# YessionCC/AR-NeRF

Measured on AMD Instinct MI355X. Metric: training rays/sec + test PSNR, Lego 8192-ray batch, 1/2/4/8 MI355X, higher is better.
Workload: dtype fp16 field (MLP forward, backward and weight gradients on fp16 MFMA operands, fp32 accumulate) / fp32 march, composite, Adam; 1 GPU; lego-shaped training step: 8192 rays/rank, scale 0.5, 1 x 128^3 grid, L=16 F=2 T=2^19 hash, 64-wide MLPs, raw loss, Adam lr 1e-2; batch_rays_per_gpu=8192, global_batch_rays=8192, pretrain_steps=2000, graphs=True, chunk_first=64, row_forward=1, march_fork=r1, parallelism=dp1, hash_backward=hybrid, bin_level_lo=8, bin_merge_hi=11, steps_per_graph_replay=2, erode=False

## Files before the change

ar-nerf_amd/csrc/hashbin.hip:

```cpp
#pragma clang fp contract(off)

#include "common.h"
#include "grid.h"

namespace ngp {

constexpr int BSHIFT = 13, BENT = 1 << BSHIFT;
constexpr int NBL = (1 << 19) / BENT;
constexpr int ACC_T = BENT / 8;
constexpr int NSLOT = L * NBL;
constexpr int MAXB = 2048;
constexpr int TILE = 256;
constexpr int RPT = TILE * 4 / 256;
constexpr uint32_t CH = 32768;
constexpr uint32_t IB_CAP = 8192;
constexpr uint32_t F_C0 = 1u << 28;
constexpr uint32_t F_SINGLE = 1u << 29;

struct BinArgs {
    int lo;
    uint32_t merge;
    uint32_t bbase[L + 1];
    int64_t tiles_cap;
};

struct BinWs {
    uint32_t* fb;
    uint32_t* tot;
    uint32_t* rstart;
    uint32_t* items;
    uint32_t* ib;
    uint32_t* ofs;
    uint4* rec;
};

static size_t align256(size_t x) { return (x + 255) & ~(size_t)255; }

static size_t bin_ws_bytes(int64_t tiles, BinWs* w, void* base) {
    const size_t o_fb = 0, o_tot = align256((MAXB + 1) * 4), o_rs = o_tot + align256(MAXB * 4),
                 o_it = o_rs + align256((MAXB + 1) * 4), o_ib = o_it + align256((MAXB + 1) * 4),
                 o_ofs = o_ib + align256(IB_CAP * 4);
    const size_t o_rec = align256(o_ofs + (size_t)tiles * NSLOT * 4);
    const size_t total = o_rec + (size_t)tiles * TILE * 4 * L * sizeof(uint4);
    if (w) {
        char* b = reinterpret_cast<char*>(base);
        w->fb = reinterpret_cast<uint32_t*>(b + o_fb);
        w->tot = reinterpret_cast<uint32_t*>(b + o_tot);
        w->rstart = reinterpret_cast<uint32_t*>(b + o_rs);
        w->items = reinterpret_cast<uint32_t*>(b + o_it);
        w->ib = reinterpret_cast<uint32_t*>(b + o_ib);
        w->ofs = reinterpret_cast<uint32_t*>(b + o_ofs);
        w->rec = reinterpret_cast<uint4*>(b + o_rec);
    }
    return total;
}

__device__ __forceinline__ void add_pair_direct(float* __restrict__ grad, uint32_t e, float w, float a0, float a1) {
    atomicAdd(grad + 2 * (size_t)e, w * a0);
    atomicAdd(grad + 2 * (size_t)e + 1, w * a1);
}

struct Rec {
    uint32_t e0, e1;
    float fx, a0, a1;
};

__device__ __forceinline__ Rec make_rec(const float in[3], float2 gd, int cy, int cz, const LevelLds& lv, int l) {
    const float sc = lv.scale[l];
    const uint32_t res = lv.res[l], size = lv.size[l];
    const bool dense = (lv.dense >> l) & 1u, pow2 = (lv.pow2 >> l) & 1u;
    float pos[3];
    uint32_t pg[3];
    level_cell(sc, in, pg, pos);
    const float wyz = (cy ? pos[1] : 1 - pos[1]) * (cz ? pos[2] : 1 - pos[2]);
    Rec r;
    r.fx = pos[0];
    r.a0 = wyz * gd.x;
    r.a1 = wyz * gd.y;
    r.e0 = corner_index(pg[0], pg[1] + cy, pg[2] + cz, res, size, dense, pow2);
    r.e1 = corner_index(pg[0] + 1, pg[1] + cy, pg[2] + cz, res, size, dense, pow2);
    return r;
}

struct RunInfo {
    bool head, longrun;
    uint64_t heads;
};
__device__ __forceinline__ RunInfo run_info(bool valid, uint32_t e0, uint32_t e1) {
    const int lane = threadIdx.x & 63;
    const uint32_t k0 = valid ? e0 : 0xffffffffu, k1 = valid ? e1 : (0xfffffff0u | (uint32_t)lane);
    const uint32_t p0 = __shfl_up(k0, 4, 64), p1 = __shfl_up(k1, 4, 64);
    RunInfo r;
    r.head = lane < 4 || !valid || p0 != k0 || p1 != k1;
    r.heads = __ballot(r.head);
    r.longrun = r.head && valid && lane + 4 < 64 && !((r.heads >> (lane + 4)) & 1ull);
    return r;
}

__device__ __forceinline__ void tile_inputs(const float* __restrict__ xyzs, const int32_t* __restrict__ sidx,
                                            const GridArgs& ga, int64_t j0, int64_t N, float in[RPT][3],
                                            bool valid[RPT]) {
    const int t = threadIdx.x;
#pragma unroll
    for (int k = 0; k < RPT; ++k) {
        const int64_t j = j0 + k * 64 + (t >> 2);
        valid[k] = j < N;
        const int64_t i = valid[k] && sidx ? (int64_t)sidx[j] : j;
        load_x01(xyzs, i, valid[k], ga, in[k]);
    }
}

__global__ void __launch_bounds__(256) hash_count_kernel(const float* __restrict__ xyzs, int64_t n,
                                                         const int64_t* __restrict__ n_dev,
                                                         const int32_t* __restrict__ sidx, GridArgs ga, BinArgs ba,
                                                         BinWs ws) {
    __shared__ LevelLds lv;
    __shared__ uint32_t cnt[NSLOT];
    NGP_PROBE_BEGIN(NGP_P_HASH_COUNT);
    load_levels(ga, lv);
    const int64_t N = ngp_capped_count(n_dev, n);
    const int64_t ntiles = min((N + TILE - 1) / TILE, ba.tiles_cap);
    const int t = threadIdx.x, yz = t & 3, cy = yz & 1, cz = yz >> 1;
    const float2 g0 = make_float2(0.f, 0.f);
    if (blockIdx.x == 0)
        for (int i = t; i <= MAXB; i += blockDim.x) ws.fb[i] = 0u;
    for (int64_t tile = blockIdx.x; tile < ntiles; tile += gridDim.x) {
        for (int i = t; i < NSLOT; i += 256) cnt[i] = 0;
        __syncthreads();
        float in[RPT][3];
        bool valid[RPT];
        tile_inputs(xyzs, sidx, ga, tile * TILE, N, in, valid);
#pragma unroll 1
        for (int l = ba.lo; l < L; ++l) {
            const bool merge = (ba.merge >> l) & 1u;
#pragma unroll
            for (int k = 0; k < RPT; ++k) {
                const Rec r = make_rec(in[k], g0, cy, cz, lv, l);
                if (merge) {
                    const RunInfo ri = run_info(valid[k], r.e0, r.e1);
                    if (!valid[k] || !ri.head) continue;
                    atomicAdd(&cnt[l * NBL + (r.e0 >> BSHIFT)], 1u);
                    if (ri.longrun) atomicAdd(&cnt[l * NBL + (r.e1 >> BSHIFT)], 1u);
                    continue;
                }
                if (!valid[k]) continue;
                atomicAdd(&cnt[l * NBL + (r.e0 >> BSHIFT)], 1u);
            }
        }
        __syncthreads();
        for (int i = t; i < NSLOT; i += 256) ws.ofs[(size_t)i * ba.tiles_cap + tile] = cnt[i];
        __syncthreads();
    }
    NGP_PROBE_END();
}

__global__ void __launch_bounds__(256) hash_scan_kernel(const int64_t* __restrict__ n_dev, int64_t n, BinArgs ba,
                                                        BinWs ws) {
    __shared__ uint32_t wsum[4];
    const int slot = blockIdx.x, l = slot / NBL, lb = slot % NBL;
    if (lb >= (int)(ba.bbase[l + 1] - ba.bbase[l])) return;
    const int64_t N = ngp_capped_count(n_dev, n);
    const int64_t ntiles = min((N + TILE - 1) / TILE, ba.tiles_cap);
    const int t = threadIdx.x, lane = t & 63, w = t >> 6;
    uint32_t carry = 0;
    for (int64_t c0 = 0; c0 < ntiles; c0 += 256) {
        const int64_t tile = c0 + t;
        uint32_t* p = ws.ofs + (size_t)slot * ba.tiles_cap + tile;
        const uint32_t v = tile < ntiles ? *p : 0u;
        uint32_t x = v;
#pragma unroll
        for (int o = 1; o < 64; o <<= 1) {
            const uint32_t y = __shfl_up(x, o, 64);
            if (lane >= o) x += y;
        }
        if (lane == 63) wsum[w] = x;
        __syncthreads();
        uint32_t before = carry;
        for (int i = 0; i < w; ++i) before += wsum[i];
        const uint32_t blk = wsum[0] + wsum[1] + wsum[2] + wsum[3];
        if (tile < ntiles) *p = before + x - v;
        carry += blk;
        __syncthreads();
    }
    if (t == 0) ws.tot[ba.bbase[l] + lb] = carry;
}

__global__ void __launch_bounds__(MAXB / 2) hash_plan_kernel(uint32_t nbt, BinWs ws) {
    __shared__ uint32_t a[MAXB / 2], c[MAXB / 2];
    NGP_PROBE_BEGIN(NGP_P_HASH_PLAN);
    const uint32_t t = threadIdx.x, b0 = 2 * t, b1 = 2 * t + 1;
    const uint32_t t0 = b0 < nbt ? ws.tot[b0] : 0u, t1 = b1 < nbt ? ws.tot[b1] : 0u;
    const uint32_t c0 = (t0 + CH - 1) / CH, c1 = (t1 + CH - 1) / CH;
    a[t] = t0 + t1;
    c[t] = c0 + c1;
    __syncthreads();
    for (uint32_t o = 1; o < MAXB / 2; o <<= 1) {
        const uint32_t va = t >= o ? a[t - o] : 0u, vc = t >= o ? c[t - o] : 0u;
        __syncthreads();
        a[t] += va;
        c[t] += vc;
        __syncthreads();
    }
    ws.rstart[b0 + 1] = a[t] - t1;
    ws.rstart[b1 + 1] = a[t];
    ws.items[b0 + 1] = c[t] - c1;
    ws.items[b1 + 1] = c[t];
    if (t == 0) { ws.rstart[0] = 0; ws.items[0] = 0; }
    for (uint32_t it = c[t] - c1 - c0; it < c[t] - c1 && it < IB_CAP; ++it) ws.ib[it] = b0;
    for (uint32_t it = c[t] - c1; it < c[t] && it < IB_CAP; ++it) ws.ib[it] = b1;
    NGP_PROBE_END();
}

template <int MODE>
__global__ void __launch_bounds__(256) hash_write_kernel(const float* __restrict__ xyzs, int64_t n,
                                                         const int64_t* __restrict__ n_dev,
                                                         const int32_t* __restrict__ sidx, GridArgs ga, BinArgs ba,
                                                         const float* __restrict__ denc, float* __restrict__ grad,
                                                         BinWs ws) {
    static_assert((MODE & 2) || NBL == 64, "MODE 0 (diagnostics) scans one wave of buckets");
    __shared__ LevelLds lv;
    __shared__ uint32_t base[NSLOT];
    __shared__ uint32_t hist2[2][NBL], loff[NBL + 1];
    __shared__ uint4 stage[TILE * 4];
    __shared__ uint8_t sbk[TILE * 4];
    uint32_t* const hall = reinterpret_cast<uint32_t*>(stage);
    static_assert(sizeof(stage) >= NSLOT * sizeof(uint32_t), "stage[] holds the per-level counters");
    NGP_PROBE_BEGIN(NGP_P_HASH_WRITE);
    load_levels(ga, lv);
    const int64_t N = ngp_capped_count(n_dev, n);
    const int64_t ntiles = (N + TILE - 1) / TILE;
    const int t = threadIdx.x, yz = t & 3, cy = yz & 1, cz = yz >> 1;
    for (int64_t tile = blockIdx.x; tile < ntiles; tile += gridDim.x) {
        const bool spill = tile >= ba.tiles_cap;
        if (spill && t == 0) ws.fb[MAXB] = 1u;
        if (!spill) {
            for (int i = t; i < NSLOT; i += 256) {
                const int l = i / NBL, lb = i % NBL;
                base[i] = lb < (int)(ba.bbase[l + 1] - ba.bbase[l])
                              ? ws.rstart[ba.bbase[l] + lb] + ws.ofs[(size_t)i * ba.tiles_cap + tile]
                              : 0u;
                if (MODE & 2) hall[i] = 0;
            }
        }
        float in[RPT][3];
        bool valid[RPT];
        const int64_t j0 = tile * TILE;
        tile_inputs(xyzs, sidx, ga, j0, N, in, valid);
        float2 gd[RPT], gn[RPT];
#pragma unroll
        for (int k = 0; k < RPT; ++k)
            gd[k] = valid[k] ? *reinterpret_cast<const float2*>(denc + (j0 + k * 64 + (t >> 2)) * 32 + 2 * ba.lo)
                             : float2{0.f, 0.f};
        if (MODE & 2) __syncthreads();
#pragma unroll 1
        for (int l = ba.lo; l < L; ++l) {
            uint32_t* hist = (MODE & 2) ? hall + l * NBL : hist2[l & 1];
            if (!(MODE & 2)) {
                if (t < NBL) hist[t] = 0;
                __syncthreads();
            }
#pragma unroll
            for (int k = 0; k < RPT; ++k)
                gn[k] = valid[k] && l + 1 < L
                            ? *reinterpret_cast<const float2*>(denc + (j0 + k * 64 + (t >> 2)) * 32 + 2 * (l + 1))
                            : float2{0.f, 0.f};
            const uint32_t off = lv.off[l];
            uint4 rec[RPT];
            uint32_t slot[RPT];
            if ((ba.merge >> l) & 1u) {
#pragma unroll
                for (int k = 0; k < RPT; ++k) {
                    const Rec r = make_rec(in[k], gd[k], cy, cz, lv, l);
                    const RunInfo ri = run_info(valid[k], r.e0, r.e1);
                    const int lane = t & 63;
                    float v00 = (1 - r.fx) * r.a0, v01 = (1 - r.fx) * r.a1, v10 = r.fx * r.a0, v11 = r.fx * r.a1;
                    if (ri.heads != ~0ull) {
#pragma unroll
                        for (int o4 = 4; o4 < 64; o4 <<= 1) {
                            const float d00 = __shfl_down(v00, o4, 64), d01 = __shfl_down(v01, o4, 64);
                            const float d10 = __shfl_down(v10, o4, 64), d11 = __shfl_down(v11, o4, 64);
                            const uint64_t span = ((0x1111111111111111ull & ((2ull << o4) - 1ull)) & ~1ull) << lane;
                            if (lane + o4 < 64 && (ri.heads & span) == 0) {
                                v00 += d00; v01 += d01; v10 += d10; v11 += d11;
                            }
                        }
                    }
                    if (!valid[k] || !ri.head) continue;
                    if (spill) {
                        atomicAdd(grad + 2 * (size_t)(off + r.e0), v00);
                        atomicAdd(grad + 2 * (size_t)(off + r.e0) + 1, v01);
                        atomicAdd(grad + 2 * (size_t)(off + r.e1), v10);
                        atomicAdd(grad + 2 * (size_t)(off + r.e1) + 1, v11);
                        continue;
                    }
                    const uint32_t b0 = r.e0 >> BSHIFT, b1 = r.e1 >> BSHIFT;
                    if (ri.longrun) {
                        const uint4 q0 = make_uint4((r.e0 & (BENT - 1)) | F_SINGLE, __float_as_uint(v00),
                                                    __float_as_uint(v01), 0u);
                        const uint4 q1 = make_uint4((r.e1 & (BENT - 1)) | F_SINGLE, __float_as_uint(v10),
                                                    __float_as_uint(v11), 0u);
                        ws.rec[base[l * NBL + b0] + atomicAdd(&hist[b0], 1u)] = q0;
                        ws.rec[base[l * NBL + b1] + atomicAdd(&hist[b1], 1u)] = q1;
                        continue;
                    }
                    uint32_t key = (r.e0 & (BENT - 1)) | ((r.e1 & (BENT - 1)) << BSHIFT);
                    if (b1 != b0) {
                        key |= F_C0;
                        add_pair_direct(grad, off + r.e1, r.fx, r.a0, r.a1);
                        ws.fb[ba.bbase[l] + b1] = 1u;
                    }
                    ws.rec[base[l * NBL + b0] + atomicAdd(&hist[b0], 1u)] =
                        make_uint4(key, __float_as_uint(r.fx), __float_as_uint(r.a0), __float_as_uint(r.a1));
                }
#pragma unroll
                for (int k = 0; k < RPT; ++k) gd[k] = gn[k];
                continue;
            }
#pragma unroll
            for (int k = 0; k < RPT; ++k) {
                slot[k] = ~0u;
                if (!valid[k]) continue;
                const Rec r = make_rec(in[k], gd[k], cy, cz, lv, l);
                if (spill) {
                    add_pair_direct(grad, off + r.e0, 1 - r.fx, r.a0, r.a1);
                    add_pair_direct(grad, off + r.e1, r.fx, r.a0, r.a1);
                    continue;
                }
                const uint32_t b0 = r.e0 >> BSHIFT, b1 = r.e1 >> BSHIFT;
                uint32_t key = (r.e0 & (BENT - 1)) | ((r.e1 & (BENT - 1)) << BSHIFT);
                if (b1 != b0) {
                    key |= F_C0;
                    add_pair_direct(grad, off + r.e1, r.fx, r.a0, r.a1);
                    ws.fb[ba.bbase[l] + b1] = 1u;
                }
                rec[k] = make_uint4(key, __float_as_uint(r.fx), __float_as_uint(r.a0), __float_as_uint(r.a1));
                slot[k] = (b0 << 16) | ((MODE & 4) ? (uint32_t)(t & 15) : atomicAdd(&hist[b0], 1u));
            }
#pragma unroll
            for (int k = 0; k < RPT; ++k) gd[k] = gn[k];
            if (spill) continue;
            if (MODE & 2) {
#pragma unroll
                for (int k = 0; k < RPT; ++k)
                    if (slot[k] != ~0u && !(MODE & 1))
                        ws.rec[base[l * NBL + (slot[k] >> 16)] + (slot[k] & 0xffffu)] = rec[k];
                continue;
            }
            __syncthreads();
            if (t < 64) {
                const uint32_t h = hist[t];
                uint32_t x = h;
#pragma unroll
                for (int o = 1; o < 64; o <<= 1) {
                    const uint32_t y = __shfl_up(x, o, 64);
                    if (t >= o) x += y;
                }
                loff[t] = x - h;
                if (t == 63) loff[NBL] = x;
            }
            __syncthreads();
#pragma unroll
            for (int k = 0; k < RPT; ++k) {
                if (slot[k] == ~0u) continue;
                const uint32_t bb = slot[k] >> 16, r = loff[bb] + (slot[k] & 0xffffu);
                stage[r] = rec[k];
                sbk[r] = (uint8_t)bb;
            }
            __syncthreads();
            const uint32_t nrec = loff[NBL];
            for (uint32_t r = t; r < nrec; r += 256) {
                const uint32_t bb = sbk[r];
                if (!(MODE & 1)) ws.rec[base[l * NBL + bb] + (r - loff[bb])] = stage[r];
                else if (stage[r].x == 0xdeadbeefu) ws.fb[0] = 2u;
            }
        }
        __syncthreads();
    }
    NGP_PROBE_END();
}

__device__ __forceinline__ bool fused_bucket(const BinWs& ws, uint32_t b, bool overflow) {
    return !overflow && ws.items[b + 1] - ws.items[b] <= 1u;
}

__device__ __forceinline__ uint32_t bucket_level(const BinArgs& ba, uint32_t b) {
    int l = 0;
    while (l < L - 1 && b >= ba.bbase[l + 1]) ++l;
    return (uint32_t)l;
}

__device__ __forceinline__ void adam4_regs(const AdamArgs& a, size_t base, uint32_t e, float4 g, float4 P, float4 M,
                                           float4 V, float lr, float bc1, float bc2) {
    adam_elem(P.x, M.x, V.x, g.x, lr, a.b1, a.b2, a.eps, bc1, bc2);
    adam_elem(P.y, M.y, V.y, g.y, lr, a.b1, a.b2, a.eps, bc1, bc2);
    adam_elem(P.z, M.z, V.z, g.z, lr, a.b1, a.b2, a.eps, bc1, bc2);
    adam_elem(P.w, M.w, V.w, g.w, lr, a.b1, a.b2, a.eps, bc1, bc2);
    reinterpret_cast<float4*>(a.p + base)[e] = P;
    reinterpret_cast<float4*>(a.m + base)[e] = M;
    reinterpret_cast<float4*>(a.v + base)[e] = V;
    typedef _Float16 h4 __attribute__((ext_vector_type(4)));
    reinterpret_cast<h4*>(a.p16 + base)[e] = h4{(_Float16)P.x, (_Float16)P.y, (_Float16)P.z, (_Float16)P.w};
}

__device__ __forceinline__ void adam4(const AdamArgs& a, size_t base, uint32_t e, float4 g, float lr, float bc1,
                                      float bc2) {
    adam4_regs(a, base, e, g, reinterpret_cast<const float4*>(a.p + base)[e],
               reinterpret_cast<const float4*>(a.m + base)[e], reinterpret_cast<const float4*>(a.v + base)[e], lr, bc1,
               bc2);
}

#ifndef NGP_ACC_PHASE
#define NGP_ACC_PHASE(k)
#endif
template <bool FUSED = false>
__global__ void __launch_bounds__(ACC_T) hash_accum_kernel(GridArgs ga, BinArgs ba, uint32_t nbt,
                                                          float* __restrict__ grad, BinWs ws, AdamArgs adam,
                                                          uint32_t b_lo, uint32_t b_hi) {
    extern __shared__ __attribute__((aligned(16))) double img[];
    NGP_PROBE_BEGIN(NGP_P_HASH_ACCUM);
    const uint32_t total = ws.items[b_hi];
    const int t = threadIdx.x, lane = t & 63;
    const bool overflow = ws.fb[MAXB] != 0;
    float lr = 0.f, bc1 = 1.f, bc2 = 1.f;
    if (FUSED) adam_bias(adam.lr_dev, adam.step_dev, adam.b1, adam.b2, lr, bc1, bc2);
    for (uint32_t it = ws.items[b_lo] + blockIdx.x; it < total; it += gridDim.x) {
        NGP_ACC_PHASE(0);
        uint32_t lo = b_lo, hi = b_hi;
        if (it < IB_CAP) {
            lo = ws.ib[it];
        } else {
            while (hi - lo > 1) {
                const uint32_t mid = (lo + hi) >> 1;
                if (ws.items[mid] <= it) lo = mid; else hi = mid;
            }
        }
        const uint32_t b = lo, c = it - ws.items[b], nch = ws.items[b + 1] - ws.items[b];
        int l = 0;
        while (l < L - 1 && b >= ba.bbase[l + 1]) ++l;
        const uint32_t lb = b - ba.bbase[l];
        const uint32_t ne = min((uint32_t)BENT, ga.g.sizes[l] - (lb << BSHIFT));
        const size_t gbase = 2 * ((size_t)ga.g.offsets[l] + ((size_t)lb << BSHIFT));
        const bool own = nch == 1 && !overflow && ws.fb[b] == 0;
        const bool fz = FUSED && nch == 1 && !overflow;
        const bool flagged = ws.fb[b] != 0;
        NGP_ACC_PHASE(1);
        const uint32_t ng = 2 * ne / 4;
        for (uint32_t e = t; e < 2 * BENT / 2; e += blockDim.x)
            reinterpret_cast<double2*>(img)[e] = make_double2(0.0, 0.0);
        __syncthreads();
        NGP_ACC_PHASE(2);
        const uint32_t r0 = ws.rstart[b] + c * CH, r1 = min(ws.rstart[b + 1], r0 + CH);
        constexpr int U = FUSED ? 2 : 4;
        uint4 v[U];
#pragma unroll
        for (int u = 0; u < U; ++u) {
            const uint32_t q = r0 + t + u * blockDim.x;
            v[u] = q < r1 ? ws.rec[q] : make_uint4(0u, 0u, 0u, 0u);
        }
        for (uint32_t q0 = r0 + t; q0 < r1; q0 += U * blockDim.x) {
            uint4 vn[U];
#pragma unroll
            for (int u = 0; u < U; ++u) {
                const uint32_t q = q0 + (U + u) * blockDim.x;
                vn[u] = q < r1 ? ws.rec[q] : make_uint4(0u, 0u, 0u, 0u);
            }
#pragma unroll
            for (int u = 0; u < U; ++u) {
                const uint32_t q = q0 + u * blockDim.x;
                const uint32_t key = v[u].x, i0 = key & (BENT - 1), i1 = (key >> BSHIFT) & (BENT - 1);
                const float fx = __uint_as_float(v[u].y), a0 = __uint_as_float(v[u].z), a1 = __uint_as_float(v[u].w);
                const float w0 = 1 - fx;
                const bool single = key & F_SINGLE;
                const bool c1 = !(key & (F_C0 | F_SINGLE));
                double p00 = single ? (double)fx : (double)(w0 * a0), p01 = single ? (double)a0 : (double)(w0 * a1);
                double p10 = c1 ? (double)(fx * a0) : 0.0, p11 = c1 ? (double)(fx * a1) : 0.0;
                const bool pad = q >= r1;
                const uint32_t kk = pad ? 0xf0000000u | lane : key;
                const uint32_t prev = __shfl_up(kk, 4, 64);
                const bool head = lane < 4 || prev != kk;
                const uint64_t heads = __ballot(head);
                if (heads != ~0ull) {
#pragma unroll
                    for (int o4 = 4; o4 < 64; o4 <<= 1) {
                        const double d00 = __shfl_down(p00, o4, 64), d01 = __shfl_down(p01, o4, 64);
                        const double d10 = __shfl_down(p10, o4, 64), d11 = __shfl_down(p11, o4, 64);
                        const uint64_t span = (0x1111111111111111ull & ((2ull << o4) - 1ull)) & ~1ull;
                        if (lane + o4 < 64 && (heads & (span << lane)) == 0) {
                            p00 += d00; p01 += d01; p10 += d10; p11 += d11;
                        }
                    }
                }
                if (!head || pad) continue;
                atomicAdd(&img[i0], p00);
                atomicAdd(&img[BENT + i0], p01);
                if (c1) {
                    atomicAdd(&img[i1], p10);
                    atomicAdd(&img[BENT + i1], p11);
                }
            }
#pragma unroll
            for (int u = 0; u < U; ++u) v[u] = vn[u];
        }
        __syncthreads();
        NGP_ACC_PHASE(3);
        float* g = grad + gbase;
        auto image4 = [&](uint32_t e) {
            const double2 f0 = reinterpret_cast<const double2*>(img)[e];
            const double2 f1 = reinterpret_cast<const double2*>(img + BENT)[e];
            return make_float4((float)f0.x, (float)f1.x, (float)f0.y, (float)f1.y);
        };
        auto fused_grad = [&](uint32_t e) {
            float4 v = image4(e);
            if (flagged) {
                float4* g4 = reinterpret_cast<float4*>(g) + e;
                const float4 m = *g4;
                v.x = m.x + v.x; v.y = m.y + v.y; v.z = m.z + v.z; v.w = m.w + v.w;
                *g4 = make_float4(0.f, 0.f, 0.f, 0.f);
            }
            const float sc = adam.grad_scale;
            return make_float4(v.x * sc, v.y * sc, v.z * sc, v.w * sc);
        };
        for (uint32_t e = t; e < ng; e += blockDim.x) {
            if (fz) {
                adam4(adam, gbase, e, fused_grad(e), lr, bc1, bc2);
                continue;
            }
            const float4 v = image4(e);
            if (own) {
                float4 o = reinterpret_cast<const float4*>(g)[e];
                o.x += v.x; o.y += v.y; o.z += v.z; o.w += v.w;
                reinterpret_cast<float4*>(g)[e] = o;
            } else {
                if (v.x != 0.f) atomicAdd(g + 4 * e, v.x);
                if (v.y != 0.f) atomicAdd(g + 4 * e + 1, v.y);
                if (v.z != 0.f) atomicAdd(g + 4 * e + 2, v.z);
                if (v.w != 0.f) atomicAdd(g + 4 * e + 3, v.w);
            }
        }
        __syncthreads();
        NGP_ACC_PHASE(4);
    }
    if (FUSED) {
        for (uint32_t b = b_lo + blockIdx.x; b < b_hi; b += gridDim.x) {
            if (ws.tot[b] != 0u || !fused_bucket(ws, b, overflow)) continue;
            const uint32_t l = bucket_level(ba, b), lb = b - ba.bbase[l];
            const uint32_t ne = min((uint32_t)BENT, ga.g.sizes[l] - (lb << BSHIFT));
            const size_t gbase = 2 * ((size_t)ga.g.offsets[l] + ((size_t)lb << BSHIFT));
            const bool flagged = ws.fb[b] != 0;
            float4* g4 = reinterpret_cast<float4*>(grad + gbase);
            for (uint32_t e = t; e < 2 * ne / 4; e += blockDim.x) {
                float4 gv = make_float4(0.f, 0.f, 0.f, 0.f);
                if (flagged) {
                    const float sc = adam.grad_scale;
                    const float4 m = g4[e];
                    gv = make_float4(m.x * sc, m.y * sc, m.z * sc, m.w * sc);
                    g4[e] = make_float4(0.f, 0.f, 0.f, 0.f);
                }
                adam4(adam, gbase, e, gv, lr, bc1, bc2);
            }
        }
    }
    NGP_PROBE_END();
}

__global__ void __launch_bounds__(256) hash_adam_residual_kernel(GridArgs ga, BinArgs ba, uint32_t nbt,
                                                                  float* __restrict__ grad, BinWs ws, AdamArgs adam,
                                                                  uint32_t b_lo) {
    NGP_PROBE_BEGIN(NGP_P_RESIDUAL);
    const uint32_t b = b_lo + blockIdx.x;
    const bool mine = b < nbt && !fused_bucket(ws, b, ws.fb[MAXB] != 0);
    float lr = 0.f, bc1 = 1.f, bc2 = 1.f;
    if (mine) adam_bias(adam.lr_dev, adam.step_dev, adam.b1, adam.b2, lr, bc1, bc2);
    if (mine) {
        const uint32_t l = bucket_level(ba, b), lb = b - ba.bbase[l];
        const uint32_t ne = min((uint32_t)BENT, ga.g.sizes[l] - (lb << BSHIFT));
        const size_t gbase = 2 * ((size_t)ga.g.offsets[l] + ((size_t)lb << BSHIFT));
        float4* g4 = reinterpret_cast<float4*>(grad + gbase);
        const float sc = adam.grad_scale;
        for (uint32_t e = threadIdx.x; e < 2 * ne / 4; e += blockDim.x) {
            const float4 gv = g4[e];
            adam4(adam, gbase, e, make_float4(gv.x * sc, gv.y * sc, gv.z * sc, gv.w * sc), lr, bc1, bc2);
            g4[e] = make_float4(0.f, 0.f, 0.f, 0.f);
        }
    }
    NGP_PROBE_END();
}

static int bin_args(const ngp_hashgrid_t* grid, int64_t tiles_cap, int lo, int merge_hi, BinArgs& ba,
                    uint32_t& nbt) {
    if (lo < 0 || lo >= L || merge_hi < 0 || merge_hi > L) return NGP_EINVAL;
    ba.lo = lo;
    ba.merge = merge_hi >= 32 ? 0xffffffffu : ((1u << merge_hi) - 1u);
    uint32_t b = 0;
    for (int l = 0; l < L; ++l) {
        ba.bbase[l] = b;
        const uint32_t nb = l < lo ? 0u : (grid->sizes[l] + BENT - 1) >> BSHIFT;
        if (nb > (uint32_t)NBL) return NGP_ERANGE;
        if (grid->offsets[l] & 1u) return NGP_EINVAL;
        b += nb;
    }
    ba.bbase[L] = b;
    ba.tiles_cap = tiles_cap;
    nbt = b;
    return b <= (uint32_t)MAXB ? NGP_OK : NGP_ERANGE;
}

}

using namespace ngp;

extern "C" {

size_t ngp_hash_backward_binned_workspace(int64_t max_samples) {
    if (max_samples <= 0) return 0;
    return bin_ws_bytes((max_samples + TILE - 1) / TILE, nullptr, nullptr);
}

static int hash_binned(const float* xyzs, int64_t n, const int64_t* n_dev, const int32_t* sample_idx,
                       const ngp_hashgrid_t* grid, const float* denc, float* grad_table, void* workspace,
                       int64_t max_samples, int level_lo, int merge_hi, int phase, void* stream,
                       const AdamArgs* adam = nullptr, int acc_lo = 0, int acc_hi = L) {
    GridArgs ga;
    int st = grid_args(grid, ga);
    if (st) return st;
    NGP_CHECK_ARG(n >= 0 && max_samples > 0);
    if (n == 0) return NGP_OK;
    NGP_CHECK_ARG(xyzs && workspace && ((uintptr_t)workspace & 255) == 0);
    if (phase & 6)
        NGP_CHECK_ARG(grad_table && ((uintptr_t)grad_table & 15) == 0);
    if (phase & 2) NGP_CHECK_ARG(denc && ((uintptr_t)denc & 7) == 0);
    const int64_t tiles_cap = (max_samples + TILE - 1) / TILE;
    NGP_CHECK_ARG(tiles_cap * TILE * 4 * L < (int64_t)0xffffffffLL);
    BinArgs ba;
    uint32_t nbt;
    st = bin_args(grid, tiles_cap, level_lo, merge_hi, ba, nbt);
    if (st) return st;
    NGP_CHECK_ARG(0 <= acc_lo && acc_lo <= acc_hi && acc_hi <= L);
    const uint32_t b_lo = ba.bbase[acc_lo], b_hi = ba.bbase[acc_hi];
    BinWs ws;
    bin_ws_bytes(tiles_cap, &ws, workspace);
    hipStream_t s = as_stream(stream);
    if (phase & 1) {
        static const unsigned capC = resident_blocks(hash_count_kernel, 256, 0);
        NGP_TIMED(NGP_K_HASH_COUNT, s, hash_count_kernel<<<persistent_blocks(n, TILE, capC), 256, 0, s>>>(xyzs, n, n_dev, sample_idx, ga, ba, ws));
        NGP_TIMED(NGP_K_HASH_SCAN, s, hash_scan_kernel<<<NSLOT, 256, 0, s>>>(n_dev, n, ba, ws));
        NGP_TIMED(NGP_K_HASH_PLAN, s, hash_plan_kernel<<<1, MAXB / 2, 0, s>>>(nbt, ws));
    }
    if (phase & 2) {
        static const unsigned capW = resident_blocks(hash_write_kernel<2>, 256, 0);
        NGP_TIMED(NGP_K_HASH_WRITE, s, hash_write_kernel<2><<<persistent_blocks(n, TILE, capW), 256, 0, s>>>(xyzs, n, n_dev, sample_idx, ga, ba,
                                                                           denc, grad_table, ws));
    }
    if (phase & 4) {
        static bool attr = false;
        const size_t lds = (size_t)BENT * 2 * sizeof(double);
        if (!attr) {
            if (hipFuncSetAttribute((const void*)hash_accum_kernel<false>, hipFuncAttributeMaxDynamicSharedMemorySize,
                                    (int)lds) != hipSuccess ||
                hipFuncSetAttribute((const void*)hash_accum_kernel<true>,
                                    hipFuncAttributeMaxDynamicSharedMemorySize, (int)lds) != hipSuccess)
                return NGP_ERANGE;
            attr = true;
        }
        static const unsigned capB = resident_blocks(hash_accum_kernel<false>, ACC_T, lds);
        if (adam) {
            NGP_TIMED(NGP_K_HASH_ACCUM, s, hash_accum_kernel<true><<<capB, ACC_T, lds, s>>>(ga, ba, nbt, grad_table, ws, *adam, b_lo, b_hi));
            if (b_hi > b_lo)
                NGP_TIMED(NGP_K_ADAM, s, hash_adam_residual_kernel<<<b_hi - b_lo, 256, 0, s>>>(ga, ba, nbt, grad_table, ws, *adam, b_lo));
        } else {
            NGP_TIMED(NGP_K_HASH_ACCUM, s, hash_accum_kernel<false><<<capB, ACC_T, lds, s>>>(ga, ba, nbt, grad_table, ws, AdamArgs{}, b_lo, b_hi));
        }
    }
    return ngp_launch_status();
}

int ngp_hash_backward_binned(const float* xyzs, int64_t n, const int64_t* n_dev, const int32_t* sample_idx,
                             const ngp_hashgrid_t* grid, const float* denc, float* grad_table, void* workspace,
                             int64_t max_samples, int level_lo, int merge_hi, void* stream) {
    return hash_binned(xyzs, n, n_dev, sample_idx, grid, denc, grad_table, workspace, max_samples, level_lo,
                       merge_hi, 7, stream);
}

int ngp_hash_binned_plan(const float* xyzs, int64_t n, const int64_t* n_dev, const int32_t* sample_idx,
                         const ngp_hashgrid_t* grid, void* workspace, int64_t max_samples, int level_lo,
                         int merge_hi, void* stream) {
    return hash_binned(xyzs, n, n_dev, sample_idx, grid, nullptr, nullptr, workspace, max_samples, level_lo,
                       merge_hi, 1, stream);
}

int ngp_hash_binned_apply(const float* xyzs, int64_t n, const int64_t* n_dev, const int32_t* sample_idx,
                          const ngp_hashgrid_t* grid, const float* denc, float* grad_table, void* workspace,
                          int64_t max_samples, int level_lo, int merge_hi, void* stream) {
    return hash_binned(xyzs, n, n_dev, sample_idx, grid, denc, grad_table, workspace, max_samples, level_lo,
                       merge_hi, 6, stream);
}

int ngp_hash_binned_write(const float* xyzs, int64_t n, const int64_t* n_dev, const int32_t* sample_idx,
                          const ngp_hashgrid_t* grid, const float* denc, float* grad_table, void* workspace,
                          int64_t max_samples, int level_lo, int merge_hi, void* stream) {
    return hash_binned(xyzs, n, n_dev, sample_idx, grid, denc, grad_table, workspace, max_samples, level_lo,
                       merge_hi, 2, stream);
}

int ngp_hash_binned_apply_adam(const float* xyzs, int64_t n, const int64_t* n_dev, const int32_t* sample_idx,
                               const ngp_hashgrid_t* grid, const float* denc, float* grad_table, void* workspace,
                               int64_t max_samples, int level_lo, int merge_hi, float* params, float* exp_avg,
                               float* exp_avg_sq, void* params_f16, const float* lr_dev, float beta1, float beta2,
                               float eps, const int64_t* step_dev, float grad_scale, void* stream) {
    NGP_CHECK_ARG(params && exp_avg && exp_avg_sq && params_f16 && lr_dev && step_dev);
    NGP_CHECK_ARG(((uintptr_t)params & 15) == 0 && ((uintptr_t)exp_avg & 15) == 0 && ((uintptr_t)exp_avg_sq & 15) == 0 &&
                  ((uintptr_t)params_f16 & 7) == 0);
    const AdamArgs a{params, exp_avg, exp_avg_sq, (_Float16*)params_f16, lr_dev, step_dev, beta1, beta2, eps,
                     grad_scale};
    return hash_binned(xyzs, n, n_dev, sample_idx, grid, denc, grad_table, workspace, max_samples, level_lo,
                       merge_hi, 6, stream, &a);
}

int ngp_hash_binned_accum_adam(const ngp_hashgrid_t* grid, float* grad_table, void* workspace, int64_t max_samples,
                               int level_lo, int merge_hi, float* params, float* exp_avg, float* exp_avg_sq,
                               void* params_f16, const float* lr_dev, float beta1, float beta2, float eps,
                               const int64_t* step_dev, float grad_scale, void* stream) {
    NGP_CHECK_ARG(params && exp_avg && exp_avg_sq && params_f16 && lr_dev && step_dev);
    NGP_CHECK_ARG(((uintptr_t)params & 15) == 0 && ((uintptr_t)exp_avg & 15) == 0 && ((uintptr_t)exp_avg_sq & 15) == 0 &&
                  ((uintptr_t)params_f16 & 7) == 0);
    const AdamArgs a{params, exp_avg, exp_avg_sq, (_Float16*)params_f16, lr_dev, step_dev, beta1, beta2, eps,
                     grad_scale};
    static const float dummy[1] = {0.f};
    return hash_binned(dummy, 1, nullptr, nullptr, grid, nullptr, grad_table, workspace, max_samples, level_lo,
                       merge_hi, 4, stream, &a);
}

int ngp_hash_binned_accum(const ngp_hashgrid_t* grid, float* grad_table, void* workspace, int64_t max_samples,
                          int level_lo, int merge_hi, void* stream) {
    static const float dummy[1] = {0.f};
    return hash_binned(dummy, 1, nullptr, nullptr, grid, nullptr, grad_table, workspace, max_samples, level_lo,
                       merge_hi, 4, stream);
}

int ngp_hash_binned_accum_levels(const ngp_hashgrid_t* grid, float* grad_table, void* workspace, int64_t max_samples,
                                 int level_lo, int merge_hi, int acc_level_lo, int acc_level_hi, void* stream) {
    static const float dummy[1] = {0.f};
    return hash_binned(dummy, 1, nullptr, nullptr, grid, nullptr, grad_table, workspace, max_samples, level_lo,
                       merge_hi, 4, stream, nullptr, acc_level_lo, acc_level_hi);
}

}
```

Before: 19.02 million rays/s.

## Transpose bin-offset layout and fuse segmented scan with plan via last-block ticket

The per-tile bin counts are stored row-major per tile (tile x compacted bucket stride) instead of slot-major across tiles. The scan becomes a two-level segmented column scan: segment totals are published, and the last block to arrive (atomic ticket) scans them and builds the plan. This removes the separate plan kernel launch and the per-slot scan blocks that mostly exited early, and only counts the populated buckets. The cost is a last-block-arrival protocol with fences, plus an extra segc read in the write kernel. It also sets waves_per_eu on the count kernel.

```diff
diff --git a/ar-nerf_amd/csrc/hashbin.hip b/ar-nerf_amd/csrc/hashbin.hip
--- a/ar-nerf_amd/csrc/hashbin.hip
+++ b/ar-nerf_amd/csrc/hashbin.hip
@@ -17,19 +17,23 @@
 constexpr uint32_t F_C0 = 1u << 28;
 constexpr uint32_t F_SINGLE = 1u << 29;
 
+constexpr int SEG = 32;
 struct BinArgs {
     int lo;
     uint32_t merge;
     uint32_t bbase[L + 1];
     int64_t tiles_cap;
+    uint32_t rs;
 };
 
 struct BinWs {
+    uint32_t* tk;
     uint32_t* fb;
     uint32_t* tot;
     uint32_t* rstart;
     uint32_t* items;
     uint32_t* ib;
+    uint32_t* segc;
     uint32_t* ofs;
     uint4* rec;
 };
@@ -37,13 +41,17 @@
 static size_t align256(size_t x) { return (x + 255) & ~(size_t)255; }
 
 static size_t bin_ws_bytes(int64_t tiles, BinWs* w, void* base) {
-    const size_t o_fb = 0, o_tot = align256((MAXB + 1) * 4), o_rs = o_tot + align256(MAXB * 4),
-                 o_it = o_rs + align256((MAXB + 1) * 4), o_ib = o_it + align256((MAXB + 1) * 4),
-                 o_ofs = o_ib + align256(IB_CAP * 4);
+    const size_t segs = (size_t)((tiles + SEG - 1) / SEG);
+    const size_t o_fb = align256(4), o_tot = o_fb + align256((MAXB + 1) * 4),
+                 o_rs = o_tot + align256(MAXB * 4), o_it = o_rs + align256((MAXB + 1) * 4),
+                 o_ib = o_it + align256((MAXB + 1) * 4), o_seg = o_ib + align256(IB_CAP * 4),
+                 o_ofs = o_seg + align256(segs * NSLOT * 4);
     const size_t o_rec = align256(o_ofs + (size_t)tiles * NSLOT * 4);
     const size_t total = o_rec + (size_t)tiles * TILE * 4 * L * sizeof(uint4);
     if (w) {
         char* b = reinterpret_cast<char*>(base);
+        w->tk = reinterpret_cast<uint32_t*>(b);
+        w->segc = reinterpret_cast<uint32_t*>(b + o_seg);
         w->fb = reinterpret_cast<uint32_t*>(b + o_fb);
         w->tot = reinterpret_cast<uint32_t*>(b + o_tot);
         w->rstart = reinterpret_cast<uint32_t*>(b + o_rs);
@@ -110,7 +118,64 @@
     }
 }
 
-__global__ void __launch_bounds__(256) hash_count_kernel(const float* __restrict__ xyzs, int64_t n,
+__device__ __forceinline__ void publish64(uint32_t* p, uint2 v) {
+    __hip_atomic_store(reinterpret_cast<unsigned long long*>(p), (unsigned long long)v.x | ((unsigned long long)v.y << 32),
+                       __ATOMIC_RELAXED, __HIP_MEMORY_SCOPE_AGENT);
+}
+__device__ __forceinline__ bool arrive_last(uint32_t* ticket, uint32_t expected, uint32_t* flag) {
+    asm volatile("s_waitcnt vmcnt(0)" ::: "memory");
+    __syncthreads();
+    if (threadIdx.x == 0) {
+        const uint32_t k = __hip_atomic_fetch_add(ticket, 1u, __ATOMIC_RELAXED, __HIP_MEMORY_SCOPE_AGENT);
+        const bool last = k + 1u == expected;
+        if (last) {
+            __builtin_amdgcn_fence(__ATOMIC_ACQUIRE, "agent");
+            asm volatile("s_waitcnt vmcnt(0)" ::: "memory");
+        }
+        *flag = last ? 1u : 0u;
+    }
+    __syncthreads();
+    return *flag != 0u;
+}
+
+__device__ __forceinline__ void build_plan(const uint32_t* tot, uint32_t* wsum, uint32_t nbt, const BinWs& ws) {
+    NGP_PROBE_BEGIN(NGP_P_HASH_PLAN);
+    const uint32_t t = threadIdx.x, lane = t & 63u, w = t >> 6;
+    uint32_t tt[4], cc[4], a = 0, c = 0;
+#pragma unroll
+    for (int k = 0; k < 4; ++k) {
+        const uint32_t b = 4 * t + k;
+        tt[k] = b < nbt ? tot[b] : 0u;
+        cc[k] = (tt[k] + CH - 1) / CH;
+        a += tt[k];
+        c += cc[k];
+    }
+    uint32_t xa = a, xc = c;
+#pragma unroll
+    for (int o = 1; o < 64; o <<= 1) {
+        const uint32_t ya = __shfl_up(xa, o, 64), yc = __shfl_up(xc, o, 64);
+        if (lane >= (uint32_t)o) { xa += ya; xc += yc; }
+    }
+    if (lane == 63 && w < 4) { wsum[w] = xa; wsum[4 + w] = xc; }
+    __syncthreads();
+    uint32_t ra = xa - a, rc = xc - c;
+    for (uint32_t i = 0; i < w && i < 4; ++i) { ra += wsum[i]; rc += wsum[4 + i]; }
+    if (t == 0) { ws.rstart[0] = 0; ws.items[0] = 0; }
+#pragma unroll
+    for (int k = 0; k < 4; ++k) {
+        const uint32_t b = 4 * t + k;
+        if (b >= nbt) break;
+        ws.tot[b] = tt[k];
+        for (uint32_t it = rc; it < rc + cc[k] && it < IB_CAP; ++it) ws.ib[it] = b;
+        ra += tt[k];
+        rc += cc[k];
+        ws.rstart[b + 1] = ra;
+        ws.items[b + 1] = rc;
+    }
+    NGP_PROBE_END();
+}
+
+__global__ void __launch_bounds__(256) __attribute__((amdgpu_waves_per_eu(8))) hash_count_kernel(const float* __restrict__ xyzs, int64_t n,
                                                          const int64_t* __restrict__ n_dev,
                                                          const int32_t* __restrict__ sidx, GridArgs ga, BinArgs ba,
                                                          BinWs ws) {
@@ -120,12 +185,15 @@
     load_levels(ga, lv);
     const int64_t N = ngp_capped_count(n_dev, n);
     const int64_t ntiles = min((N + TILE - 1) / TILE, ba.tiles_cap);
+    const uint32_t nbt = ba.bbase[L];
     const int t = threadIdx.x, yz = t & 3, cy = yz & 1, cz = yz >> 1;
     const float2 g0 = make_float2(0.f, 0.f);
-    if (blockIdx.x == 0)
+    if (blockIdx.x == 0) {
         for (int i = t; i <= MAXB; i += blockDim.x) ws.fb[i] = 0u;
+        if (t == 0) ws.tk[0] = 0u;
+    }
     for (int64_t tile = blockIdx.x; tile < ntiles; tile += gridDim.x) {
-        for (int i = t; i < NSLOT; i += 256) cnt[i] = 0;
+        for (uint32_t i = t; i < nbt; i += 256) cnt[i] = 0;
         __syncthreads();
         float in[RPT][3];
         bool valid[RPT];
@@ -133,82 +201,94 @@
 #pragma unroll 1
         for (int l = ba.lo; l < L; ++l) {
             const bool merge = (ba.merge >> l) & 1u;
+            uint32_t* const cl = cnt + ba.bbase[l];
 #pragma unroll
             for (int k = 0; k < RPT; ++k) {
                 const Rec r = make_rec(in[k], g0, cy, cz, lv, l);
                 if (merge) {
                     const RunInfo ri = run_info(valid[k], r.e0, r.e1);
                     if (!valid[k] || !ri.head) continue;
-                    atomicAdd(&cnt[l * NBL + (r.e0 >> BSHIFT)], 1u);
-                    if (ri.longrun) atomicAdd(&cnt[l * NBL + (r.e1 >> BSHIFT)], 1u);
+                    atomicAdd(&cl[r.e0 >> BSHIFT], 1u);
+                    if (ri.longrun) atomicAdd(&cl[r.e1 >> BSHIFT], 1u);
                     continue;
                 }
                 if (!valid[k]) continue;
-                atomicAdd(&cnt[l * NBL + (r.e0 >> BSHIFT)], 1u);
+                atomicAdd(&cl[r.e0 >> BSHIFT], 1u);
             }
         }
         __syncthreads();
-        for (int i = t; i < NSLOT; i += 256) ws.ofs[(size_t)i * ba.tiles_cap + tile] = cnt[i];
+        uint32_t* const row = ws.ofs + (size_t)tile * ba.rs;
+        for (uint32_t i = t; i < nbt; i += 256) row[i] = cnt[i];
         __syncthreads();
     }
     NGP_PROBE_END();
 }
 
-__global__ void __launch_bounds__(256) hash_scan_kernel(const int64_t* __restrict__ n_dev, int64_t n, BinArgs ba,
-                                                        BinWs ws) {
-    __shared__ uint32_t wsum[4];
-    const int slot = blockIdx.x, l = slot / NBL, lb = slot % NBL;
-    if (lb >= (int)(ba.bbase[l + 1] - ba.bbase[l])) return;
+constexpr int SCAN_T = 512, SCAN_G = SCAN_T / 256;
+__device__ __forceinline__ void scan_rows(uint32_t* rows, uint32_t rs, uint32_t nrows, uint32_t* tot,
+                                          uint2 (*part)[NSLOT / 2]) {
+    const uint32_t c = threadIdx.x & 255u, q = threadIdx.x >> 8, rs2 = rs / 2;
+    for (uint32_t cb = 0; cb < rs2; cb += 256) {
+        const bool on = cb + c < rs2;
+        uint2* const col = reinterpret_cast<uint2*>(rows) + cb + c;
+        uint2 carry = make_uint2(0u, 0u);
+        for (uint32_t r0 = 0; r0 < nrows; r0 += 8 * SCAN_G) {
+            const uint32_t ra = r0 + q * 8;
+            uint2 v[8], sum = make_uint2(0u, 0u);
+#pragma unroll
+            for (uint32_t k = 0; k < 8; ++k) {
+                v[k] = on && ra + k < nrows ? col[(size_t)(ra + k) * rs2] : make_uint2(0u, 0u);
+                sum.x += v[k].x;
+                sum.y += v[k].y;
+            }
+            __syncthreads();
+            if (on) part[q][cb + c] = sum;
+            __syncthreads();
+            uint2 run = carry;
+#pragma unroll
+            for (uint32_t g = 0; g < (uint32_t)SCAN_G; ++g) {
+                const uint2 p = on ? part[g][cb + c] : make_uint2(0u, 0u);
+                if (g < q) { run.x += p.x; run.y += p.y; }
+                carry.x += p.x;
+                carry.y += p.y;
+            }
+#pragma unroll
+            for (uint32_t k = 0; k < 8; ++k) {
+                if (on && ra + k < nrows) col[(size_t)(ra + k) * rs2] = run;
+                run.x += v[k].x;
+                run.y += v[k].y;
+            }
+        }
+        if (on && q == 0) { tot[2 * (cb + c)] = carry.x; tot[2 * (cb + c) + 1] = carry.y; }
+    }
+    __syncthreads();
+}
+
+__global__ void __launch_bounds__(SCAN_T) hash_scan_kernel(const int64_t* __restrict__ n_dev, int64_t n, BinArgs ba,
+                                                           BinWs ws) {
+    __shared__ uint32_t tot[NSLOT];
+    __shared__ uint2 part[SCAN_G][NSLOT / 2];
+    __shared__ uint32_t wsum[8], lastf;
     const int64_t N = ngp_capped_count(n_dev, n);
-    const int64_t ntiles = min((N + TILE - 1) / TILE, ba.tiles_cap);
-    const int t = threadIdx.x, lane = t & 63, w = t >> 6;
-    uint32_t carry = 0;
-    for (int64_t c0 = 0; c0 < ntiles; c0 += 256) {
-        const int64_t tile = c0 + t;
-        uint32_t* p = ws.ofs + (size_t)slot * ba.tiles_cap + tile;
-        const uint32_t v = tile < ntiles ? *p : 0u;
-        uint32_t x = v;
-#pragma unroll
-        for (int o = 1; o < 64; o <<= 1) {
-            const uint32_t y = __shfl_up(x, o, 64);
-            if (lane >= o) x += y;
-        }
-        if (lane == 63) wsum[w] = x;
+    const int64_t ntiles = max((int64_t)0, min((N + TILE - 1) / TILE, ba.tiles_cap));
+    const uint32_t nseg = (uint32_t)((ntiles + SEG - 1) / SEG);
+    const uint32_t nbt = ba.bbase[L], rs = ba.rs, t = threadIdx.x;
+    if (nseg == 0 && blockIdx.x == 0) {
+        for (uint32_t i = t; i < NSLOT; i += SCAN_T) tot[i] = 0;
         __syncthreads();
-        uint32_t before = carry;
-        for (int i = 0; i < w; ++i) before += wsum[i];
-        const uint32_t blk = wsum[0] + wsum[1] + wsum[2] + wsum[3];
-        if (tile < ntiles) *p = before + x - v;
-        carry += blk;
+        build_plan(tot, wsum, nbt, ws);
+    }
+    for (uint32_t seg = blockIdx.x; seg < nseg; seg += gridDim.x) {
+        const uint32_t seg_tiles = (uint32_t)min((int64_t)SEG, ntiles - (int64_t)seg * SEG);
+        scan_rows(ws.ofs + (size_t)seg * SEG * rs, rs, seg_tiles, tot, part);
+        for (uint32_t c = t; c < rs / 2; c += SCAN_T)
+            publish64(ws.segc + (size_t)seg * rs + 2 * c, make_uint2(tot[2 * c], tot[2 * c + 1]));
+        if (arrive_last(ws.tk, nseg, &lastf)) {
+            scan_rows(ws.segc, rs, nseg, tot, part);
+            build_plan(tot, wsum, nbt, ws);
+        }
         __syncthreads();
     }
-    if (t == 0) ws.tot[ba.bbase[l] + lb] = carry;
-}
-
-__global__ void __launch_bounds__(MAXB / 2) hash_plan_kernel(uint32_t nbt, BinWs ws) {
-    __shared__ uint32_t a[MAXB / 2], c[MAXB / 2];
-    NGP_PROBE_BEGIN(NGP_P_HASH_PLAN);
-    const uint32_t t = threadIdx.x, b0 = 2 * t, b1 = 2 * t + 1;
-    const uint32_t t0 = b0 < nbt ? ws.tot[b0] : 0u, t1 = b1 < nbt ? ws.tot[b1] : 0u;
-    const uint32_t c0 = (t0 + CH - 1) / CH, c1 = (t1 + CH - 1) / CH;
-    a[t] = t0 + t1;
-    c[t] = c0 + c1;
-    __syncthreads();
-    for (uint32_t o = 1; o < MAXB / 2; o <<= 1) {
-        const uint32_t va = t >= o ? a[t - o] : 0u, vc = t >= o ? c[t - o] : 0u;
-        __syncthreads();
-        a[t] += va;
-        c[t] += vc;
-        __syncthreads();
-    }
-    ws.rstart[b0 + 1] = a[t] - t1;
-    ws.rstart[b1 + 1] = a[t];
-    ws.items[b0 + 1] = c[t] - c1;
-    ws.items[b1 + 1] = c[t];
-    if (t == 0) { ws.rstart[0] = 0; ws.items[0] = 0; }
-    for (uint32_t it = c[t] - c1 - c0; it < c[t] - c1 && it < IB_CAP; ++it) ws.ib[it] = b0;
-    for (uint32_t it = c[t] - c1; it < c[t] && it < IB_CAP; ++it) ws.ib[it] = b1;
-    NGP_PROBE_END();
 }
 
 template <int MODE>
@@ -234,11 +314,10 @@
         const bool spill = tile >= ba.tiles_cap;
         if (spill && t == 0) ws.fb[MAXB] = 1u;
         if (!spill) {
+            const uint32_t* const segc = ws.segc + (size_t)(tile / SEG) * ba.rs;
+            const uint32_t* const ofs = ws.ofs + (size_t)tile * ba.rs;
             for (int i = t; i < NSLOT; i += 256) {
-                const int l = i / NBL, lb = i % NBL;
-                base[i] = lb < (int)(ba.bbase[l + 1] - ba.bbase[l])
-                              ? ws.rstart[ba.bbase[l] + lb] + ws.ofs[(size_t)i * ba.tiles_cap + tile]
-                              : 0u;
+                if (i < (int)ba.bbase[L]) base[i] = ws.rstart[i] + segc[i] + ofs[i];
                 if (MODE & 2) hall[i] = 0;
             }
         }
@@ -265,6 +344,7 @@
                             ? *reinterpret_cast<const float2*>(denc + (j0 + k * 64 + (t >> 2)) * 32 + 2 * (l + 1))
                             : float2{0.f, 0.f};
             const uint32_t off = lv.off[l];
+            const uint32_t* const basel = base + ba.bbase[l];
             uint4 rec[RPT];
             uint32_t slot[RPT];
             if ((ba.merge >> l) & 1u) {
@@ -299,8 +379,8 @@
                                                     __float_as_uint(v01), 0u);
                         const uint4 q1 = make_uint4((r.e1 & (BENT - 1)) | F_SINGLE, __float_as_uint(v10),
                                                     __float_as_uint(v11), 0u);
-                        ws.rec[base[l * NBL + b0] + atomicAdd(&hist[b0], 1u)] = q0;
-                        ws.rec[base[l * NBL + b1] + atomicAdd(&hist[b1], 1u)] = q1;
+                        ws.rec[basel[b0] + atomicAdd(&hist[b0], 1u)] = q0;
+                        ws.rec[basel[b1] + atomicAdd(&hist[b1], 1u)] = q1;
                         continue;
                     }
                     uint32_t key = (r.e0 & (BENT - 1)) | ((r.e1 & (BENT - 1)) << BSHIFT);
@@ -309,7 +389,7 @@
                         add_pair_direct(grad, off + r.e1, r.fx, r.a0, r.a1);
                         ws.fb[ba.bbase[l] + b1] = 1u;
                     }
-                    ws.rec[base[l * NBL + b0] + atomicAdd(&hist[b0], 1u)] =
+                    ws.rec[basel[b0] + atomicAdd(&hist[b0], 1u)] =
                         make_uint4(key, __float_as_uint(r.fx), __float_as_uint(r.a0), __float_as_uint(r.a1));
                 }
 #pragma unroll
@@ -343,7 +423,7 @@
 #pragma unroll
                 for (int k = 0; k < RPT; ++k)
                     if (slot[k] != ~0u && !(MODE & 1))
-                        ws.rec[base[l * NBL + (slot[k] >> 16)] + (slot[k] & 0xffffu)] = rec[k];
+                        ws.rec[basel[(slot[k] >> 16)] + (slot[k] & 0xffffu)] = rec[k];
                 continue;
             }
             __syncthreads();
@@ -370,7 +450,7 @@
             const uint32_t nrec = loff[NBL];
             for (uint32_t r = t; r < nrec; r += 256) {
                 const uint32_t bb = sbk[r];
-                if (!(MODE & 1)) ws.rec[base[l * NBL + bb] + (r - loff[bb])] = stage[r];
+                if (!(MODE & 1)) ws.rec[basel[bb] + (r - loff[bb])] = stage[r];
                 else if (stage[r].x == 0xdeadbeefu) ws.fb[0] = 2u;
             }
         }
@@ -601,6 +681,7 @@
     }
     ba.bbase[L] = b;
     ba.tiles_cap = tiles_cap;
+    ba.rs = (b + 31u) & ~31u;
     nbt = b;
     return b <= (uint32_t)MAXB ? NGP_OK : NGP_ERANGE;
 }
@@ -643,8 +724,8 @@
     if (phase & 1) {
         static const unsigned capC = resident_blocks(hash_count_kernel, 256, 0);
         NGP_TIMED(NGP_K_HASH_COUNT, s, hash_count_kernel<<<persistent_blocks(n, TILE, capC), 256, 0, s>>>(xyzs, n, n_dev, sample_idx, ga, ba, ws));
-        NGP_TIMED(NGP_K_HASH_SCAN, s, hash_scan_kernel<<<NSLOT, 256, 0, s>>>(n_dev, n, ba, ws));
-        NGP_TIMED(NGP_K_HASH_PLAN, s, hash_plan_kernel<<<1, MAXB / 2, 0, s>>>(nbt, ws));
+        const int64_t segs = ((n + TILE - 1) / TILE + SEG - 1) / SEG;
+        NGP_TIMED(NGP_K_HASH_SCAN, s, hash_scan_kernel<<<(unsigned)min(segs, (int64_t)1024), SCAN_T, 0, s>>>(n_dev, n, ba, ws));
     }
     if (phase & 2) {
         static const unsigned capW = resident_blocks(hash_write_kernel<2>, 256, 0);
```

New measurement: 18.82 million rays/s. -1.1%, worse.
